# Const-me/Whisper

Measured on AMD Instinct MI355X. Metric: audio-seconds/sec (real-time factor), ggml-medium & large, 30s chunks @1/2/4/8 GPU, higher is better.
Workload: dtype f16

## Files before the change

### whisper_amd/binding.py

```python
from __future__ import annotations

import ctypes as C
import os
from typing import Optional, Sequence

import numpy as np

from . import ggml_format as gf

_HERE = os.path.dirname(os.path.abspath(__file__))
LIB_PATH = os.path.join(_HERE, "lib", "libwhisper_hip.so")

WH_FLAG_PARITY_PV = 1
WH_FLAG_NO_GRAPH = 2
WH_FLAG_DEBUG_CAPTURE = 4
WH_FLAG_PARITY_EXACT = 8
TUNE_GEMM_8WAVE = 16
TUNE_GEMM_4WAVE = 4
TUNE_GEMM_FAST_EPI = 1
TUNE_GEMV_ROWS4, TUNE_GEMM_BIG, TUNE_GEMV_SMALLREG, TUNE_GEMM_GL, TUNE_LN_SEPARATE_BIGM, TUNE_ATTN_XCD = 2, 8, 32, 64, 128, 256
TUNE_ATTN_DEC_G, TUNE_FUSE_CROSS_Q, TUNE_GEMM_GROUP_M, TUNE_FUSE_SELF_BLOCK, TUNE_GEMV_LN_BLOCK, TUNE_GEMV_K8 = 512, 1024, 2048, 4096, 8192, 16384
TUNE_SPLIT_STREAMS, TUNE_ATTN_ENC_F, TUNE_GEMM_WIDE_EPI, TUNE_GEMM_FRAGPF, TUNE_ATTN_ENC_2SWEEP = 32768, 65536, 131072, 262144, 524288
TUNE_GEMV_ALLROWS, TUNE_GEMV_ROWGROUPS, TUNE_SELF_MFMA, TUNE_MEL_MFMA = 1048576, 2097152, 4194304, 8388608
TUNE_DECODE_SMALL, TUNE_DECODE_PREFETCH, TUNE_ATTN_DEC_NT, TUNE_ENC_SERIAL = 16777216, 33554432, 67108864, 134217728
# ... 82 lines not shown
        if os.environ.get("WH_TUNING"):
            L.wh_debug_set_tuning(int(os.environ["WH_TUNING"], 0))
        L.wh_device_info.argtypes = [i32, C.c_char_p, C.c_size_t, C.POINTER(C.c_uint64), C.POINTER(C.c_int)]
        L.wh_model_arena_bytes.restype = i64
        L.wh_model_arena_bytes.argtypes = [C.POINTER(HParamsC)]
        L.wh_model_create.argtypes = [C.POINTER(HParamsC), vp, i32, C.POINTER(vp)]
        L.wh_model_destroy.argtypes = [vp]
        L.wh_model_destroy.restype = None
        L.wh_model_set_tensor.argtypes = [vp, C.c_char_p, i32, C.POINTER(C.c_int32), i32, vp]
        L.wh_model_set_filters.argtypes = [vp, i32, i32, vp]
        L.wh_model_finalize.argtypes = [vp]
        L.wh_model_arena.argtypes = [vp, C.POINTER(vp), C.POINTER(i64)]
        L.wh_model_hparams.argtypes = [vp, C.POINTER(HParamsC)]
        L.wh_context_create.argtypes = [vp, i32, vp, C.POINTER(vp)]
        L.wh_context_create_hyp.argtypes = [vp, i32, i32, vp, C.POINTER(vp)]
        L.wh_context_bind.argtypes = [vp]
        L.wh_context_destroy.argtypes = [vp]
        L.wh_context_destroy.restype = None
        L.wh_context_set_flags.argtypes = [vp, C.c_uint32, i32]
        L.wh_context_set_audio_ctx.argtypes = [vp, i32]
        L.wh_context_memory.argtypes = [vp, C.POINTER(i64)]
        L.wh_context_synchronize.argtypes = [vp]
        L.wh_buffer_upload_async.argtypes = [vp, vp, vp, i64]
        L.wh_mel_spectrogram.argtypes = [vp, vp, i64, vp, C.POINTER(i64)]
        L.wh_encode.argtypes = [vp, vp, i32, i64, i64, vp]
        L.wh_encode_windows.argtypes = [vp, vp, i32]
        L.wh_decode.argtypes = [vp, vp, i32, i32, i32, vp, vp]
        L.wh_sample_best.argtypes = [vp, i32, i32, i32, C.POINTER(TokenDataC)]
        L.wh_beam_candidates.argtypes = [vp, i32, i32, i32, i32, C.POINTER(TokenDataC)]
        L.wh_reorder_self_cache.argtypes = [vp, i32, vp, i32]
        L.wh_debug_read.argtypes = [vp, C.c_char_p, i32, i32, vp, i64]
        L.wh_decode_greedy.argtypes = [vp, i32, vp, i32, i32, i32, i32, C.POINTER(TokenDataC)]
        L.wh_decode_window_start.argtypes = [vp, i32, vp, i32, i32, i32, i32]
        L.wh_decode_window_finish.argtypes = [vp, C.POINTER(TokenDataC)]
        L.wh_decode_window_start_ragged.argtypes = [vp, i32, vp, vp, i32, i32, i32, i32]
        L.wh_decode_window_ready.argtypes = [vp, i32, i32]
        L.wh_decode_window_continue.argtypes = [vp, i32]
        L.wh_decode_window_fetch.argtypes = [vp, i32, i32, C.POINTER(TokenDataC)]
        L.wh_mel_spectrogram_window.argtypes = [vp, vp, i64, i64, i64, i64, i32, vp]
        L.wh_mel_spectrogram_batch.argtypes = [vp, vp, i64, i64, i32, vp, i64]
        L.wh_debug_probe.argtypes = [vp, i32, i32, i32, i32, i32, i32, C.POINTER(C.c_float)]
        L.wh_profile_enable.argtypes = [vp, i32]
        L.wh_profile_read.argtypes = [vp, C.POINTER(ProfileEntryC), i32, C.POINTER(i32)]
        L.wh_op_mul_mat.argtypes = [vp, vp, vp, vp, vp, vp, i32, i32, i32]
        L.wh_op_mul_mat_gelu.argtypes = [vp, vp, vp, vp, vp, i32, i32, i32]
        L.wh_op_layer_norm.argtypes = [vp, vp, vp, vp, vp, i32, i32]
        L.wh_op_flash_attention.argtypes = [vp, vp, vp, vp, vp, i32, i32, i32]
        L.wh_op_soft_max.argtypes = [vp, vp, i32, i32]
        L.wh_op_decoder_attention.argtypes = [vp, vp, vp, vp, vp, i32, i32, i32, i32, i32, i32, i32, i32, i32]
        L.wh_op_decoder_cross_attention.argtypes = [vp, vp, vp, vp, vp, vp, C.c_float, vp, vp, vp, i32, i32, i32, i32, i32]
        L.wh_op_vocab_soft_max.argtypes = [vp, vp, vp, i32, i32]
        L.wh_op_sample_best.argtypes = [vp, vp, i32, i32, i32, i32, i32, i32, i32, i32, vp]
        L.wh_op_beam_candidates.argtypes = [vp, vp, i32, i32, i32, i32, i32, i32, i32, i32, i32, vp]
        L.wh_op_reorder_self_cache.argtypes = [vp, vp, vp, vp, vp, vp, vp, i32, i32, i32, i32, i32, i32]
        L.wh_lang_detect.argtypes = [vp, i32, vp, vp]
        L.wh_model_lang_count.argtypes = [vp]
        L.wh_op_lang_probs.argtypes = [vp, vp, i32, i32, i32, i32, vp, vp]
        L.wh_resample_out_len.argtypes = [i32, i64, C.POINTER(i64)]
        L.wh_resample.argtypes = [vp, vp, i32, i32, i32, i32, i64, vp, i64, i64]
        L.wh_resample_host.argtypes = [vp, i32, i32, i32, i32, i64, vp, i64, i64]
        L.wh_resample_host_multi.argtypes = [vp, i32, i32, vp, i32, i32, i64, vp, vp, i64]
        L.wh_resample_taps.argtypes = [i32, C.POINTER(C.c_int32), C.POINTER(C.c_int32), C.POINTER(C.c_int32), C.POINTER(C.c_int32), vp, i64]
        L.wh_vad_frame_count.argtypes = [i64, C.POINTER(i64)]
        L.wh_vad_features.argtypes = [vp, vp, i64, vp]
        L.wh_vad_features_host.argtypes = [vp, i64, vp]
        L.wh_dequantize.argtypes = [vp, i32, vp, i64, vp]
        L.wh_model_set_alignment_heads.argtypes = [vp, vp, i32]
        L.wh_align_tokens.argtypes = [vp, i32, vp, vp, vp, i32, vp]
        L.wh_op_align_matrix.argtypes = [vp, vp, i64, i32, vp, i64, i32, i32, i32, vp, i32, vp, vp, i32, i32, i32, vp, vp]
        L.wh_op_dtw.argtypes = [vp, vp, i32, i32, i32, vp, vp, vp]
        _lib = L
    return _lib


def check(rc: int):
    if rc != 0:
        raise WhisperHipError("libwhisper_hip rc=%d: %s" % (rc, lib().wh_last_error().decode(errors="replace")))


def set_option(name: str, value: int):
    check(lib().wh_debug_set_option(name.encode(), int(value)))


OPTION_DEFAULTS = {"dec_tile": 0, "dec_depth": 0, "dec_wide_rows": 1, "dec_deep_rows": 0, "vocab_decrows": 0, "enc_chunk": 128, "self_fuse_max_rows": 32, "self_nq": 0, "self_wave_min_rows": 32, "enc_exp": 5, "exact_enc_layers": -1, "exact_alt_order": 0, "gemm_mf16": 1, "dec_lds": 1, "dec_lds_ks": 2, "dec_split": 1, "cross_mfma": 1, "vocab_lds": 1, "beam_regs": 1, "reorder_group": 1, "gemm_big_min_rows": 8192, "resample_lds_phases": 853}


def get_option(name: str) -> int:
    v = C.c_int(0)
    check(lib().wh_debug_get_option(name.encode(), C.byref(v)))
    return v.value


def get_option_default(name: str) -> int:
    return OPTION_DEFAULTS[name]


def device_count() -> int:
    return lib().wh_device_count()


def device_info(device: int = 0):
    name = C.create_string_buffer(256)
    mem = C.c_uint64()
    cus = C.c_int()
    check(lib().wh_device_info(device, name, 256, C.byref(mem), C.byref(cus)))
    return dict(name=name.value.decode(), total_mem=mem.value, compute_units=cus.value)


def _hp_c(hp: gf.HParams) -> HParamsC:
    return HParamsC(*hp.as_list())


def arena_bytes(hp: gf.HParams) -> int:
    n = lib().wh_model_arena_bytes(C.byref(_hp_c(hp)))
    if n < 0:
        check(-1)
    return int(n)


class HipModel:

    def __init__(self, hp: gf.HParams, arena_ptr: int = 0, already_filled: bool = False, keepalive=None):
        self.hp = hp
        self.handle = C.c_void_p()
        self._keepalive = keepalive
        check(lib().wh_model_create(C.byref(_hp_c(hp)), C.c_void_p(arena_ptr) if arena_ptr else None, int(already_filled),
                                    C.byref(self.handle)))

    @classmethod
    def from_ggml(cls, model: gf.GgmlModel, arena_ptr: int = 0, keepalive=None) -> "HipModel":
        m = cls(model.hparams, arena_ptr, False, keepalive)
        L = lib()
        filt = np.ascontiguousarray(model.filters, np.float32)
        check(L.wh_model_set_filters(m.handle, filt.shape[0], filt.shape[1], filt.ctypes.data_as(C.c_void_p)))
        for name, a in model.tensors.items():
            if isinstance(a, gf.QTensor):
                blocks = np.ascontiguousarray(a.blocks, np.uint8)
                ne = (C.c_int32 * len(a.shape))(*reversed(a.shape))
                check(L.wh_model_set_tensor(m.handle, name.encode(), len(a.shape), ne, gf.GGML_TYPES[a.qtype], blocks.ctypes.data_as(C.c_void_p)))
                continue
            a = np.ascontiguousarray(a)
            ne = (C.c_int32 * a.ndim)(*reversed(a.shape))
            check(L.wh_model_set_tensor(m.handle, name.encode(), a.ndim, ne, int(a.dtype == np.float16), a.ctypes.data_as(C.c_void_p)))
        check(L.wh_model_finalize(m.handle))
        return m

    @classmethod
    def from_file(cls, path: str) -> "HipModel":
        return cls.from_ggml(gf.read_model(path))

    def lang_count(self) -> int:
        n = lib().wh_model_lang_count(self.handle)
        if n < 0:
            check(n)
        return n

    def set_alignment_heads(self, pairs):
        a = np.ascontiguousarray(pairs, np.int32).reshape(-1, 2)
        check(lib().wh_model_set_alignment_heads(self.handle, a.ctypes.data_as(C.c_void_p) if len(a) else None, len(a)))

    def arena(self):
        p = C.c_void_p()
        n = C.c_int64()
        check(lib().wh_model_arena(self.handle, C.byref(p), C.byref(n)))
        return p.value, n.value

    def close(self):
# ... 327 lines not shown
```

### whisper_amd/csrc/attn_enc.hip

```cpp
#include "kernels.h"
#include <type_traits>

namespace wh
{
	namespace
	{
		constexpr int AQ = 64;
		constexpr int AWAVES = 8;
		constexpr int QSTRIDE = 72;
		constexpr int OSTRIDE = 65;
		constexpr int ATT_LDS_BYTES = AQ * QSTRIDE * 2 + 2 * AWAVES * AQ * 4 + AWAVES * AQ * 8 + 4 * AQ * OSTRIDE * 4;

		template<int KT>
		__global__ void __launch_bounds__( 512, 2 ) attentionEnc( const f16* __restrict__ q, const f16* __restrict__ k,
			const f16* __restrict__ vT, f16* __restrict__ out, int heads, int T, int Tpad, int nQ, int xcdRemap )
		{
			extern __shared__ __attribute__( ( aligned( 16 ) ) ) unsigned char smem[];
			f16* const ldsQ = (f16*)smem;
			float* const redMax = (float*)( smem + AQ * QSTRIDE * 2 );
			float* const redInv = redMax + AWAVES * AQ;
			double* const redSum = (double*)( redInv + AWAVES * AQ );
			float* const obuf = (float*)( redSum + AWAVES * AQ );

			const int tid = threadIdx.x;
// ... 594 lines not shown
			issueV( 0, 0 );
			for( int t = 0; t < nTiles; t++ )
			{
				const int buf = t & 1;
				asm volatile( "s_waitcnt vmcnt(0)" ::: "memory" );
				__syncthreads();
				if( t + 1 < nTiles )
				{
					issueK( t + 1, buf ^ 1 );
					issueV( t + 1, buf ^ 1 );
				}
				const f16* const kt = ldsK + buf * F_TILE;
				const f16* const vt = ldsV + buf * F_TILE;
	#pragma unroll
				for( int st = 0; st < 4; st++ )
				{
					const f32x16 S = scores( kt, st, t );
					f16x8 P[ 2 ];
	#pragma unroll
					for( int r = 0; r < 16; r += 2 )
					{
						typedef _Float16 h2 __attribute__( ( ext_vector_type( 2 ) ) );
						typedef unsigned short u16x2 __attribute__( ( ext_vector_type( 2 ) ) );
						const h2 hd = { (f16)( S[ r ] - mx ), (f16)( S[ r + 1 ] - mx ) };
						if constexpr( MODE == 0 )
						{
							u16x2 mag = __builtin_bit_cast( u16x2, __builtin_bit_cast( unsigned, hd ) & 0x7FFF7FFFu );
							const u16x2 lim = { (unsigned short)EXP_TABLE_LIMIT, (unsigned short)EXP_TABLE_LIMIT };
							mag = __builtin_elementwise_min( mag, lim );
							P[ r >> 3 ][ r & 7 ] = ldsTab[ mag[ 0 ] ];
							P[ r >> 3 ][ ( r & 7 ) + 1 ] = ldsTab[ mag[ 1 ] ];
						}
						else
						{
							typedef float f2 __attribute__( ( ext_vector_type( 2 ) ) );
							constexpr float L2E = 1.44269504088896340736f;
							const h2 hp = __builtin_convertvector( f2{ S[ r ] - mx, S[ r + 1 ] - mx }, h2 );
							const f2 e = { __builtin_amdgcn_exp2f( __builtin_fmaf( (float)hp[ 0 ], L2E, 0.0f ) ), __builtin_amdgcn_exp2f( __builtin_fmaf( (float)hp[ 1 ], L2E, 0.0f ) ) };
							const h2 eh = __builtin_convertvector( e, h2 );
							P[ r >> 3 ][ r & 7 ] = eh[ 0 ];
							P[ r >> 3 ][ ( r & 7 ) + 1 ] = eh[ 1 ];
						}
					}
					sum += (double)sumP( P );
	#pragma unroll
					for( int half = 0; half < 2; half++ )
					{
						const int kb = st * 2 + half;
	#pragma unroll
						for( int ddt = 0; ddt < 2; ddt++ )
						{
							const f16x8 vf = *(const f16x8*)( vt + ( ( kb * 2 + ddt ) * 64 + lane ) * 8 );
							O[ ddt ] = __builtin_amdgcn_mfma_f32_32x32x16_f16( vf, P[ half ], O[ ddt ], 0, 0, 0 );
						}
					}
				}
			}
			sum += __shfl_xor( sum, 32, 64 );
			const float invSum = (float)( 1.0 / sum );
	#pragma unroll
			for( int a = 0; a < 2; a++ )
	#pragma unroll
				for( int r = 0; r < 16; r++ ) O[ a ][ r ] *= invSum;
			if( qRow < T )
			{
				const int b = bh / heads, h = bh - b * heads;
				f16* const o = out + ( (long long)b * T + qRow ) * ( heads * HEAD_DIM ) + h * HEAD_DIM;
	#pragma unroll
				for( int ddt = 0; ddt < 2; ddt++ )
	#pragma unroll
					for( int g4 = 0; g4 < 4; g4++ )
					{
						f16x4 pk;
	#pragma unroll
						for( int e = 0; e < 4; e++ ) pk[ e ] = (f16)O[ ddt ][ 4 * g4 + e ];
						*(f16x4*)( o + ddt * 32 + 8 * g4 + 4 * hi ) = pk;
					}
			}
		}

		constexpr int W_NBUF = 4;
		constexpr int W_LDS_BYTES = 2 * W_NBUF * F_TILE * 2;
		constexpr float W_LAZY = 4.0f;
		template<int NG, bool ONLINE, bool NOARG = false>
		__global__ void __launch_bounds__( 1024 / NG, NG == 1 ? 4 : 2 ) attentionEncW( const f16* __restrict__ q, const f16* __restrict__ k,
			const f16* __restrict__ vT, f16* __restrict__ out, int heads, int T, int Tpad, int nQ, int xcdRemap )
		{
			extern __shared__ __attribute__( ( aligned( 16 ) ) ) unsigned char smemW[];
			f16* const ldsK = (f16*)smemW;
			f16* const ldsV = ldsK + W_NBUF * F_TILE;
			typedef __attribute__( ( address_space( 3 ) ) ) void* LdsPtr;
			typedef const __attribute__( ( address_space( 1 ) ) ) void* GlobalPtr;
			typedef _Float16 h2 __attribute__( ( ext_vector_type( 2 ) ) );
			typedef float f2 __attribute__( ( ext_vector_type( 2 ) ) );
			constexpr float L2E = 1.44269504088896340736f;

			const int tid = threadIdx.x;
			const int lane = tid & 63;
			const int wave = tid >> 6;
			const int hi = lane >> 5;
			const int c = lane & 31;
			int bh, qb;
			{
				const int L = blockIdx.x;
				if( xcdRemap )
				{
					const int kIdx = L >> 3;
					bh = ( L & 7 ) + 8 * ( kIdx / nQ );
					qb = kIdx % nQ;
				}
				else
				{
					bh = L / nQ;
					qb = L - bh * nQ;
				}
			}
			const f16* const Q = q + (long long)bh * T * HEAD_DIM;
			const f16* const K = k + (long long)bh * T * HEAD_DIM;
			const f16* const VT = vT + (long long)bh * HEAD_DIM * Tpad;
			const int nTiles = ( T + FK - 1 ) / FK;
			int qRow[ NG ];
			f16x8 qf[ NG ][ 4 ];
	#pragma unroll
			for( int g = 0; g < NG; g++ )
			{
				qRow[ g ] = qb * TQ + ( wave * NG + g ) * 32 + c;
				const int qr = qRow[ g ] < T ? qRow[ g ] : T - 1;
	#pragma unroll
				for( int kk = 0; kk < 4; kk++ )
				{
					qf[ g ][ kk ] = *(const f16x8*)( Q + (long long)qr * HEAD_DIM + kk * 16 + hi * 8 );
	#pragma unroll
					for( int j = 0; j < 8; j++ ) qf[ g ][ kk ][ j ] = qf[ g ][ kk ][ j ] * (f16)0.125f;
				}
			}
			auto issueK = [ & ]( int t, int buf )
			{
	#pragma unroll
				for( int i = 0; i < NG; i++ )
				{
					const int row = ( wave * NG + i ) * 8 + ( lane >> 3 );
					const int cl = ( lane & 7 ) ^ ( ( row >> 1 ) & 7 );
					int key = t * FK + row;
					key = key < T ? key : T - 1;
					__builtin_amdgcn_global_load_lds( (GlobalPtr)( K + (long long)key * HEAD_DIM + cl * 8 ),
						(LdsPtr)( ldsK + buf * F_TILE + ( wave * NG + i ) * 512 ), 16, 0, 0 );
				}
			};
			auto issueV = [ & ]( int t, int buf )
			{
	#pragma unroll
				for( int i = 0; i < NG; i++ )
					__builtin_amdgcn_global_load_lds( (GlobalPtr)( VT + (long long)t * F_TILE + ( wave * NG + i ) * 512 + lane * 8 ),
						(LdsPtr)( ldsV + buf * F_TILE + ( wave * NG + i ) * 512 ), 16, 0, 0 );
			};
			auto waitTile = [ & ]( int t, auto per )
			{
				constexpr int P = decltype( per )::value;
				const int younger = min( W_NBUF - 2, nTiles - 1 - t );
				if( younger >= 2 )
				{
					if constexpr( P == 2 ) asm volatile( "s_waitcnt vmcnt(4)" ::: "memory" );
					else asm volatile( "s_waitcnt vmcnt(8)" ::: "memory" );
				}
				else if( younger == 1 )
				{
					if constexpr( P == 2 ) asm volatile( "s_waitcnt vmcnt(2)" ::: "memory" );
// ... 29 lines not shown
			auto sumP = [ & ]( const f16x8 ( &P )[ 2 ] ) -> float
			{
				const h2 ones = { (f16)1.0f, (f16)1.0f };
				float part = 0.0f;
	#pragma unroll
				for( int h = 0; h < 2; h++ )
	#pragma unroll
					for( int j = 0; j < 8; j += 2 )
						part = __builtin_amdgcn_fdot2( h2{ P[ h ][ j ], P[ h ][ j + 1 ] }, ones, part, false );
				return part;
			};
			auto expTile = [ & ]( const f32x16& S, float mref, f16x8 ( &P )[ 2 ] )
			{
	#pragma unroll
				for( int r = 0; r < 16; r += 2 )
				{
					f2 e;
					if constexpr( NOARG )
					{
						const float mL = mref * L2E;
						e = f2{ __builtin_amdgcn_exp2f( __builtin_fmaf( S[ r ], L2E, -mL ) ), __builtin_amdgcn_exp2f( __builtin_fmaf( S[ r + 1 ], L2E, -mL ) ) };
					}
					else
					{
						const h2 hd = __builtin_convertvector( f2{ S[ r ] - mref, S[ r + 1 ] - mref }, h2 );
						e = f2{ __builtin_amdgcn_exp2f( __builtin_fmaf( (float)hd[ 0 ], L2E, 0.0f ) ), __builtin_amdgcn_exp2f( __builtin_fmaf( (float)hd[ 1 ], L2E, 0.0f ) ) };
					}
					const h2 eh = __builtin_convertvector( e, h2 );
					P[ r >> 3 ][ r & 7 ] = eh[ 0 ];
					P[ r >> 3 ][ ( r & 7 ) + 1 ] = eh[ 1 ];
				}
			};

			float mx[ NG ];
	#pragma unroll
			for( int g = 0; g < NG; g++ ) mx[ g ] = -INFINITY;
			if constexpr( !ONLINE )
			{
	#pragma unroll
				for( int i = 0; i < W_NBUF - 1; i++ )
					if( i < nTiles ) issueK( i, i );
				for( int t = 0; t < nTiles; t++ )
				{
					waitTile( t, std::integral_constant<int, NG>{} );
					__syncthreads();
					if( t + W_NBUF - 1 < nTiles ) issueK( t + W_NBUF - 1, ( t + W_NBUF - 1 ) % W_NBUF );
					const f16* const kt = ldsK + ( t % W_NBUF ) * F_TILE;
					auto body = [ & ]( auto last )
					{
	#pragma unroll
						for( int st = 0; st < 4; st++ )
						{
							f32x16 S[ NG ];
							scores( kt, st, t, last, S );
	#pragma unroll
							for( int g = 0; g < NG; g++ )
	#pragma unroll
								for( int r = 0; r < 16; r++ ) mx[ g ] = fmaxf( mx[ g ], S[ g ][ r ] );
						}
					};
					if( t == nTiles - 1 ) body( std::true_type{} ); else body( std::false_type{} );
				}
	#pragma unroll
				for( int g = 0; g < NG; g++ ) mx[ g ] = fmaxf( mx[ g ], __shfl_xor( mx[ g ], 32, 64 ) );
				__syncthreads();
			}

			double sum[ NG ];
			float sumF[ NG ];
			f32x16 O[ NG ][ 2 ];
	#pragma unroll
			for( int g = 0; g < NG; g++ )
			{
				sum[ g ] = 0.0;
				sumF[ g ] = 0.0f;
	#pragma unroll
				for( int a = 0; a < 2; a++ )
	#pragma unroll
					for( int r = 0; r < 16; r++ ) O[ g ][ a ][ r ] = 0.0f;
			}
	#pragma unroll
			for( int i = 0; i < W_NBUF - 1; i++ )
				if( i < nTiles ) { issueK( i, i ); issueV( i, i ); }
			for( int t = 0; t < nTiles; t++ )
			{
				waitTile( t, std::integral_constant<int, 2 * NG>{} );
				__syncthreads();
				if( t + W_NBUF - 1 < nTiles )
				{
					issueK( t + W_NBUF - 1, ( t + W_NBUF - 1 ) % W_NBUF );
					issueV( t + W_NBUF - 1, ( t + W_NBUF - 1 ) % W_NBUF );
				}
				const f16* const kt = ldsK + ( t % W_NBUF ) * F_TILE;
				const f16* const vt = ldsV + ( t % W_NBUF ) * F_TILE;
				auto body = [ & ]( auto last )
				{
	#pragma unroll
					for( int st = 0; st < 4; st++ )
					{
						f32x16 S[ NG ];
						scores( kt, st, t, last, S );
						if constexpr( ONLINE )
						{
							float tm[ NG ];
							bool raise = false;
	#pragma unroll
							for( int g = 0; g < NG; g++ )
							{
								tm[ g ] = S[ g ][ 0 ];
	#pragma unroll
								for( int r = 1; r < 16; r++ ) tm[ g ] = fmaxf( tm[ g ], S[ g ][ r ] );
								tm[ g ] = fmaxf( tm[ g ], __shfl_xor( tm[ g ], 32, 64 ) );
								raise = raise || tm[ g ] > mx[ g ] + W_LAZY;
							}
							if( __any( raise ) )
							{
	#pragma unroll
								for( int g = 0; g < NG; g++ )
								{
									const float mNew = tm[ g ] > mx[ g ] + W_LAZY ? tm[ g ] : mx[ g ];
									const float f = __builtin_amdgcn_exp2f( ( mx[ g ] - mNew ) * L2E );
									mx[ g ] = mNew;
									sumF[ g ] *= f;
	#pragma unroll
									for( int a = 0; a < 2; a++ )
	#pragma unroll
										for( int r = 0; r < 16; r++ ) O[ g ][ a ][ r ] *= f;
								}
							}
						}
						f16x8 P[ NG ][ 2 ];
	#pragma unroll
						for( int g = 0; g < NG; g++ )
						{
							expTile( S[ g ], mx[ g ], P[ g ] );
							if constexpr( ONLINE ) sumF[ g ] += sumP( P[ g ] );
							else sum[ g ] += (double)sumP( P[ g ] );
						}
	#pragma unroll
						for( int half = 0; half < 2; half++ )
						{
							const int kb = st * 2 + half;
	#pragma unroll
							for( int ddt = 0; ddt < 2; ddt++ )
							{
								const f16x8 vf = *(const f16x8*)( vt + ( ( kb * 2 + ddt ) * 64 + lane ) * 8 );
	#pragma unroll
								for( int g = 0; g < NG; g++ ) O[ g ][ ddt ] = __builtin_amdgcn_mfma_f32_32x32x16_f16( vf, P[ g ][ half ], O[ g ][ ddt ], 0, 0, 0 );
							}
						}
					}
				};
				if( t == nTiles - 1 ) body( std::true_type{} ); else body( std::false_type{} );
			}
	#pragma unroll
			for( int g = 0; g < NG; g++ )
			{
				if constexpr( ONLINE ) sum[ g ] = (double)sumF[ g ];
				sum[ g ] += __shfl_xor( sum[ g ], 32, 64 );
				const float invSum = (float)( 1.0 / sum[ g ] );
				if( qRow[ g ] < T )
				{
					const int b = bh / heads, h = bh - b * heads;
					f16* const o = out + ( (long long)b * T + qRow[ g ] ) * ( heads * HEAD_DIM ) + h * HEAD_DIM;
	#pragma unroll
					for( int ddt = 0; ddt < 2; ddt++ )
	#pragma unroll
						for( int g4 = 0; g4 < 4; g4++ )
						{
							f16x4 pk;
	#pragma unroll
							for( int e = 0; e < 4; e++ ) pk[ e ] = (f16)( O[ g ][ ddt ][ 4 * g4 + e ] * invSum );
							*(f16x4*)( o + ddt * 32 + 8 * g4 + 4 * hi ) = pk;
						}
				}
			}
		}

		template<int NG, bool ONLINE, bool NOARG = false>
		int launchEncWideT( const f16* q, const f16* k, const f16* vT, f16* out, int batch, int heads, int T, int Tpad, hipStream_t stream )
		{
			static PerDeviceOnce once;
			if( const int onceDev = once.needed(); onceDev >= 0 )
			{
				WH_HIP( hipFuncSetAttribute( (const void*)attentionEncW<NG, ONLINE, NOARG>, hipFuncAttributeMaxDynamicSharedMemorySize, W_LDS_BYTES ) );
				once.mark( onceDev );
			}
			const int nQ = ( T + TQ - 1 ) / TQ, BH = batch * heads;
			const int xcdRemap = ( BH % 8 ) == 0 && ( g_tuning & TUNE_ATTN_XCD ) ? 1 : 0;
			hipLaunchKernelGGL( ( attentionEncW<NG, ONLINE, NOARG> ), dim3( nQ * BH ), dim3( 1024 / NG ), W_LDS_BYTES, stream, q, k, vT, out, heads, T, Tpad, nQ, xcdRemap );
			WH_HIP( hipGetLastError() );
			return 0;
		}
		int launchEncWide( const f16* q, const f16* k, const f16* vT, f16* out, int batch, int heads, int T, int Tpad, int mode, hipStream_t stream )
		{
			if( mode == 5 ) return launchEncWideT<2, true, true>( q, k, vT, out, batch, heads, T, Tpad, stream );
			if( mode == 3 ) return launchEncWideT<2, true>( q, k, vT, out, batch, heads, T, Tpad, stream );
			return launchEncWideT<2, false>( q, k, vT, out, batch, heads, T, Tpad, stream );
		}

		int launchEncTable( const f16* q, const f16* k, const f16* vT, f16* out, int batch, int heads, int T, int Tpad, const f16* expTab, hipStream_t stream )
		{
			static PerDeviceOnce once;
			if( const int onceDev = once.needed(); onceDev >= 0 )
			{
				WH_HIP( hipFuncSetAttribute( (const void*)attentionEncT<0>, hipFuncAttributeMaxDynamicSharedMemorySize, T_LDS_BYTES ) );
				WH_HIP( hipFuncSetAttribute( (const void*)attentionEncT<1>, hipFuncAttributeMaxDynamicSharedMemorySize, T_LDS_BYTES - T_TABLE_HALFS * 2 ) );
				once.mark( onceDev );
			}
			const int nQ = ( T + TQ - 1 ) / TQ, BH = batch * heads;
			const int xcdRemap = ( BH % 8 ) == 0 && ( g_tuning & TUNE_ATTN_XCD ) ? 1 : 0;
			if( g_opt.encExp == 2 || g_opt.encExp == 3 || g_opt.encExp == 5 ) return launchEncWide( q, k, vT, out, batch, heads, T, Tpad, g_opt.encExp, stream );
			if( g_opt.encExp == 1 )
				hipLaunchKernelGGL( attentionEncT<1>, dim3( nQ * BH ), dim3( 1024 ), T_LDS_BYTES - T_TABLE_HALFS * 2, stream, q, k, vT, out, expTab, heads, T, Tpad, nQ, xcdRemap );
			else
			hipLaunchKernelGGL( attentionEncT<0>, dim3( nQ * BH ), dim3( 1024 ), T_LDS_BYTES, stream, q, k, vT, out, expTab, heads, T, Tpad, nQ, xcdRemap );
			WH_HIP( hipGetLastError() );
			return 0;
		}

		int launchEncF( const f16* q, const f16* k, const f16* vT, f16* out, int batch, int heads, int T, int Tpad, bool exactP, hipStream_t stream )
		{
			static PerDeviceOnce once;
			if( const int onceDev = once.needed(); onceDev >= 0 )
			{
				WH_HIP( hipFuncSetAttribute( (const void*)attentionEncF<false>, hipFuncAttributeMaxDynamicSharedMemorySize, F_LDS_BYTES ) );
				WH_HIP( hipFuncSetAttribute( (const void*)attentionEncF<true>, hipFuncAttributeMaxDynamicSharedMemorySize, F_LDS_BYTES ) );
				once.mark( onceDev );
			}
			const int nQ = ( T + FQ - 1 ) / FQ, BH = batch * heads;
			const int xcdRemap = ( BH % 8 ) == 0 && ( g_tuning & TUNE_ATTN_XCD ) ? 1 : 0;
			const bool two = !exactP && ( g_tuning & TUNE_ATTN_ENC_2SWEEP );
			if( two )
				hipLaunchKernelGGL( attentionEncF<true>, dim3( nQ * BH ), dim3( 512 ), F_LDS_BYTES, stream, q, k, vT, out, heads, T, Tpad, nQ, xcdRemap );
			else
				hipLaunchKernelGGL( attentionEncF<false>, dim3( nQ * BH ), dim3( 512 ), F_LDS_BYTES, stream, q, k, vT, out, heads, T, Tpad, nQ, xcdRemap );
			WH_HIP( hipGetLastError() );
			return 0;
		}

		template<int KT>
		int launchEncT( const f16* q, const f16* k, const f16* vT, f16* out, int batch, int heads, int T, int Tpad, hipStream_t stream )
		{
			static PerDeviceOnce once;
			if( const int onceDev = once.needed(); onceDev >= 0 )
			{
				WH_HIP( hipFuncSetAttribute( (const void*)attentionEnc<KT>, hipFuncAttributeMaxDynamicSharedMemorySize, ATT_LDS_BYTES ) );
				once.mark( onceDev );
			}
			const int nQ = ( T + AQ - 1 ) / AQ, BH = batch * heads;
			const int xcdRemap = ( BH % 8 ) == 0 && ( g_tuning & TUNE_ATTN_XCD ) ? 1 : 0;
			hipLaunchKernelGGL( attentionEnc<KT>, dim3( nQ * BH ), dim3( 512 ), ATT_LDS_BYTES, stream, q, k, vT, out, heads, T, Tpad, nQ, xcdRemap );
			WH_HIP( hipGetLastError() );
			return 0;
		}
	}

	int attentionInit() { return 0; }

	int launchAttentionEnc( const f16* q, const f16* k, const f16* vT, f16* out, int batch, int heads, int T, int Tpad, bool exactP, const f16* expTab,
		hipStream_t stream )
	{
		if( T <= 0 || T > 1536 || Tpad < ( ( T + 255 ) / 256 ) * 256 || ( Tpad & 7 ) != 0 )
		{
			setError( "attentionEnc: need 0 < T <= 1536 and Tpad >= roundup(T, 256)" );
			return -1;
		}
		if( expTab && !exactP && ( g_tuning & TUNE_ATTN_ENC_TABLE ) && ( g_tuning & TUNE_ATTN_ENC_F ) && ( g_tuning & TUNE_ATTN_ENC_2SWEEP ) &&
			( ( ( T + TQ - 1 ) / TQ ) * batch * heads >= 256 || ( g_tuning & TUNE_ATTN_ENC_TABLE_ANY ) ) )
			return launchEncTable( q, k, vT, out, batch, heads, T, Tpad, expTab, stream );
		if( g_tuning & TUNE_ATTN_ENC_F ) return launchEncF( q, k, vT, out, batch, heads, T, Tpad, exactP, stream );
		switch( ( T + 255 ) / 256 )
		{
		case 1: return launchEncT<1>( q, k, vT, out, batch, heads, T, Tpad, stream );
		case 2: return launchEncT<2>( q, k, vT, out, batch, heads, T, Tpad, stream );
		case 3: return launchEncT<3>( q, k, vT, out, batch, heads, T, Tpad, stream );
		case 4: return launchEncT<4>( q, k, vT, out, batch, heads, T, Tpad, stream );
		case 5: return launchEncT<5>( q, k, vT, out, batch, heads, T, Tpad, stream );
// ... 5 lines not shown
```

### whisper_amd/csrc/kernels.h

```cpp
#pragma once
#include "common.h"

namespace wh
{
	enum eTuning : unsigned
	{
		TUNE_GEMV_ROWS4 = 2,
		TUNE_GEMM_4WAVE = 4,
		TUNE_GEMM_FAST_EPI = 1,
		TUNE_GEMM_8WAVE = 16,
		TUNE_GEMM_BIG = 8,
		TUNE_GEMV_SMALLREG = 32,
		TUNE_GEMM_GL = 64,
		TUNE_LN_SEPARATE_BIGM = 128,
		TUNE_ATTN_XCD = 256,
		TUNE_ATTN_DEC_G = 512,
		TUNE_FUSE_CROSS_Q = 1024,
		TUNE_FUSE_SELF_BLOCK = 4096,
		TUNE_GEMV_LN_BLOCK = 8192,
		TUNE_GEMV_K8 = 16384,
		TUNE_SPLIT_STREAMS = 32768,
		TUNE_ATTN_ENC_F = 65536,
		TUNE_GEMM_WIDE_EPI = 131072,
		TUNE_GEMM_FRAGPF = 262144,
		TUNE_ATTN_ENC_2SWEEP = 524288,
		TUNE_MEL_MFMA = 8388608,
		TUNE_SELF_MFMA = 4194304,
		TUNE_GEMV_ALLROWS = 1048576,
		TUNE_GEMV_ROWGROUPS = 2097152,
		TUNE_GEMM_GROUP_M = 2048,
		TUNE_ATTN_DEC_NT = 67108864,
		TUNE_DECODE_SMALL = 16777216,
		TUNE_DECODE_PREFETCH = 33554432,
		TUNE_ATTN_ENC_TABLE = 268435456,
		TUNE_ATTN_ENC_TABLE_ANY = 1073741824,
		TUNE_SAMPLE_SPREAD = 2147483648u,
		TUNE_GEMV_MT8 = 536870912,
		TUNE_ENC_SERIAL = 134217728,
		TUNE_DEFAULT = TUNE_GEMM_FAST_EPI | TUNE_GEMM_8WAVE | TUNE_GEMV_ROWS4 | TUNE_GEMV_SMALLREG | TUNE_GEMM_BIG | TUNE_GEMM_GL | TUNE_LN_SEPARATE_BIGM | TUNE_ATTN_XCD | TUNE_ATTN_DEC_G | TUNE_FUSE_CROSS_Q | TUNE_GEMM_GROUP_M | TUNE_FUSE_SELF_BLOCK | TUNE_GEMV_K8 | TUNE_ATTN_ENC_F | TUNE_GEMM_WIDE_EPI | TUNE_GEMM_FRAGPF | TUNE_ATTN_ENC_2SWEEP | TUNE_GEMV_ALLROWS | TUNE_GEMV_ROWGROUPS | TUNE_SELF_MFMA | TUNE_MEL_MFMA | TUNE_DECODE_SMALL | TUNE_ATTN_DEC_NT | TUNE_ATTN_ENC_TABLE
	};
	extern unsigned g_tuning;

	struct Options
	{
		int decTile = 0;
		int decDepth = 0;
		int decWideRows = 1;
		int decDeepRows = 0;
		int vocabDecRows = 0;
		int encChunk = 128;
		int selfFuseMaxRows = 32;
		int selfNq = 0;
		int exactEncLayers = -1;
		int encExp = 5;
		int encAblate = 0;
		int exactAltOrder = 0;
		int decLds = 1;
		int decLdsKs = 2;
		int decSplit = 1;
		int crossMfma = 1;
		int vocabLds = 1;
		int beamRegs = 1;
		int reorderGroup = 1;
		int gemmBigMinRows = 8192;
		int gemmMf16 = 1;
		int resampleLdsPhases = 853;
		int selfWaveMinRows = 32;
	};
	extern Options g_opt;

	enum eEpilogue : int
	{
		EPI_F32 = 0,
		EPI_F16_GELU,
		EPI_CONV2,
		EPI_QKV_ENC,
		EPI_CROSS_KV,
		EPI_QKV_DEC,
		EPI_Q_DEC,
	};

	struct GemmArgs
	{
		const f16* A;
		const f16* W;
		int M, N, K;
		int lda, Mb;
		long long aBatchStride;
		int epi;
		const float* bias;
		const float* res;
		float* out32;
		f16* out16;
		int ldc;
		long long cBatchStride;
		const float* pe;
		float scale;
		f16* q;
		f16* k;
		f16* v;
		int T, Tpad, H, B;
		int nTok, nPast, textCtx;
		const int* nPastDev;
		const float* lnX;
		const float* lnW;
		const float* lnB;
		int wideEpi;
		int groupM;
		float* splitScratch;
		int cuLimit;
	};

	int launchGemm( const GemmArgs& a, hipStream_t stream );
	int launchGemmSkinny( const GemmArgs& a, hipStream_t stream );
	int launchGemv( const GemmArgs& a, hipStream_t stream );
	constexpr int GEMV_FUSED_MAX_ROWS = 128;
	constexpr int GEMV_MAX_ROWS = 512;
	int launchGemmVariant( const GemmArgs& a, int variant, hipStream_t stream );
	int gemmInit();

	int launchLayerNorm( const float* x, const float* w, const float* b, f16* out, int rows, int d, hipStream_t stream );
	struct MelWindow
	{
		const float* mel;
		long long len;
		int offset, reserved;
	};
	int launchMelToConvInput( const float* mel, long long melStride, long long melLen, const int* melOffsets, const MelWindow* wins,
		f16* x16, long long xBatchStride, int nMels, int T, int batch, hipStream_t stream );
	int launchEmbed( const int* tokens, const f16* te, const float* pe, float* x, int rows, int nTok, int nPast, const int* nPastDev, int d,
		int nVocab, int nTextCtx, hipStream_t stream );
	int launchSoftMaxRows( float* x, int rows, int cols, hipStream_t stream );

	int launchExactMulMat( const f16* W, int N, int K, const float* X, long long ldx, int M, float* out, long long ldo, const float* bias, float scale, bool useScale,
		const f16* geluTab, const float* residual, long long ldr, hipStream_t stream );
	int launchExactNorm( const float* x, const float* w, const float* b, float* out, int rows, int n, hipStream_t stream );
	int launchExactConv( const f16* W, int kpad, int ic, const void* X, bool in16, long long xBatchStride, int Tin, int stride, const float* bias, const f16* geluTab,
// ... 176 lines not shown
```

### whisper_amd/csrc/options.hip

```cpp
#include "runtime.h"

namespace wh
{
	unsigned g_tuning = TUNE_DEFAULT;
	Options g_opt;
	namespace
	{
		struct OptionName { const char* name; int Options::* field; };
		const OptionName g_optionNames[] = { { "dec_tile", &Options::decTile }, { "dec_depth", &Options::decDepth }, { "dec_wide_rows", &Options::decWideRows }, { "dec_deep_rows", &Options::decDeepRows }, { "vocab_decrows", &Options::vocabDecRows }, { "enc_chunk", &Options::encChunk },
			{ "self_fuse_max_rows", &Options::selfFuseMaxRows }, { "self_nq", &Options::selfNq }, { "self_wave_min_rows", &Options::selfWaveMinRows }, { "exact_enc_layers", &Options::exactEncLayers }, { "exact_alt_order", &Options::exactAltOrder }, { "enc_exp", &Options::encExp }, { "enc_ablate", &Options::encAblate }, { "gemm_mf16", &Options::gemmMf16 }, { "dec_lds", &Options::decLds }, { "dec_lds_ks", &Options::decLdsKs }, { "dec_split", &Options::decSplit }, { "vocab_lds", &Options::vocabLds }, { "beam_regs", &Options::beamRegs }, { "reorder_group", &Options::reorderGroup }, { "gemm_big_min_rows", &Options::gemmBigMinRows }, { "cross_mfma", &Options::crossMfma }, { "resample_lds_phases", &Options::resampleLdsPhases } };
		const bool g_optionsFromEnv = []()
		{
			for( const OptionName& o : g_optionNames )
			{
				std::string env = "WH_OPT_";
				for( const char* p = o.name; *p; p++ ) env.push_back( (char)toupper( (unsigned char)*p ) );
				if( const char* e = getenv( env.c_str() ) )
				{
					char* end = nullptr;
					const long v = strtol( e, &end, 10 );
					if( end != e && *end == 0 && v >= -1 && v <= ( 1 << 24 ) ) g_opt.*( o.field ) = (int)v;
					else fprintf( stderr, "[wh] %s='%s' ignored (not an integer in [-1, 2^24])\n", env.c_str(), e );
				}
			}
			return true;
		}();
	}
	static thread_local std::string g_lastError;
	void setError( const std::string& s ) { g_lastError = s; }
	int hipFail( hipError_t e, const char* what, const char* file, int line )
	{
		char buf[ 512 ];
		snprintf( buf, sizeof( buf ), "HIP error %d (%s) at %s:%d: %s", (int)e, hipGetErrorString( e ), file, line, what );
		g_lastError = buf;
		return WH_E_HIP;
	}
}

extern "C" {

const char* wh_last_error( void ) { return g_lastError.c_str(); }

int wh_debug_set_tuning( uint32_t mask )
{
	g_tuning = mask;
	return 0;
}

int wh_debug_set_option( const char* name, int value )
{
	if( !name ) { setError( "debug_set_option: null name" ); return WH_E_INVALIDARG; }
	for( const OptionName& o : g_optionNames )
		if( 0 == strcmp( o.name, name ) )
		{
			if( value < -1 || value > ( 1 << 24 ) ) { setError( std::string( "option '" ) + name + "': value out of range" ); return WH_E_INVALIDARG; }
			g_opt.*( o.field ) = value;
			return 0;
		}
	setError( "debug_set_option: unknown option" );
	return WH_E_INVALIDARG;
}

int wh_debug_get_option( const char* name, int* value )
{
	if( !name || !value ) { setError( "debug_get_option: null argument" ); return WH_E_INVALIDARG; }
	for( const OptionName& o : g_optionNames )
		if( 0 == strcmp( o.name, name ) )
		{
			*value = g_opt.*( o.field );
			return 0;
		}
	setError( "debug_get_option: unknown option" );
	return WH_E_INVALIDARG;
}

}
```

Measured before the change: 10440.

## Add software-pipelined encoder attention loop with K-fragment double buffering

Adds a SCHED=1 variant of the wide encoder attention kernel that reads the next sub-tile's K fragments from LDS while the current sub-tile's score MFMAs and softmax run, with V fragments loaded early and sched_barriers pinning the instruction order. It also exits early on the last tile once the valid sub-tiles are done, instead of computing masked ones. The aim is to hide LDS latency behind MFMA work in the encoder attention. The variant is on by default through a new enc_sched option, which costs extra registers for the double-buffered fragments and hand-written asm for the rescale step.

After: 10580 (median of 6 runs). +1.3%, better.

```diff
diff --git a/whisper_amd/binding.py b/whisper_amd/binding.py
--- a/whisper_amd/binding.py
+++ b/whisper_amd/binding.py
@@ -188,7 +188,7 @@
     check(lib().wh_debug_set_option(name.encode(), int(value)))
 
 
-OPTION_DEFAULTS = {"dec_tile": 0, "dec_depth": 0, "dec_wide_rows": 1, "dec_deep_rows": 0, "vocab_decrows": 0, "enc_chunk": 128, "self_fuse_max_rows": 32, "self_nq": 0, "self_wave_min_rows": 32, "enc_exp": 5, "exact_enc_layers": -1, "exact_alt_order": 0, "gemm_mf16": 1, "dec_lds": 1, "dec_lds_ks": 2, "dec_split": 1, "cross_mfma": 1, "vocab_lds": 1, "beam_regs": 1, "reorder_group": 1, "gemm_big_min_rows": 8192, "resample_lds_phases": 853}
+OPTION_DEFAULTS = {"dec_tile": 0, "dec_depth": 0, "dec_wide_rows": 1, "dec_deep_rows": 0, "vocab_decrows": 0, "enc_chunk": 128, "self_fuse_max_rows": 32, "self_nq": 0, "self_wave_min_rows": 32, "enc_exp": 5, "enc_sched": 1, "exact_enc_layers": -1, "exact_alt_order": 0, "gemm_mf16": 1, "dec_lds": 1, "dec_lds_ks": 2, "dec_split": 1, "cross_mfma": 1, "vocab_lds": 1, "beam_regs": 1, "reorder_group": 1, "gemm_big_min_rows": 8192, "resample_lds_phases": 853}
 
 
 def get_option(name: str) -> int:
diff --git a/whisper_amd/csrc/attn_enc.hip b/whisper_amd/csrc/attn_enc.hip
--- a/whisper_amd/csrc/attn_enc.hip
+++ b/whisper_amd/csrc/attn_enc.hip
@@ -700,7 +700,7 @@
 		constexpr int W_NBUF = 4;
 		constexpr int W_LDS_BYTES = 2 * W_NBUF * F_TILE * 2;
 		constexpr float W_LAZY = 4.0f;
-		template<int NG, bool ONLINE, bool NOARG = false>
+		template<int NG, bool ONLINE, bool NOARG = false, int SCHED = 0>
 		__global__ void __launch_bounds__( 1024 / NG, NG == 1 ? 4 : 2 ) attentionEncW( const f16* __restrict__ q, const f16* __restrict__ k,
 			const f16* __restrict__ vT, f16* __restrict__ out, int heads, int T, int Tpad, int nQ, int xcdRemap )
 		{
@@ -896,6 +896,114 @@
 	#pragma unroll
 			for( int i = 0; i < W_NBUF - 1; i++ )
 				if( i < nTiles ) { issueK( i, i ); issueV( i, i ); }
+			if constexpr( SCHED == 1 )
+			{
+				static_assert( ONLINE && NG == 2, "the scheduled loop is the one-sweep form of two query groups per wave" );
+				const int swK = ( c >> 1 ) & 7;
+				auto tile = [ & ]( int t, auto last )
+				{
+					waitTile( t, std::integral_constant<int, 2 * NG>{} );
+					__syncthreads();
+					if( t + W_NBUF - 1 < nTiles )
+					{
+						issueK( t + W_NBUF - 1, ( t + W_NBUF - 1 ) % W_NBUF );
+						issueV( t + W_NBUF - 1, ( t + W_NBUF - 1 ) % W_NBUF );
+					}
+					const f16* const kt = ldsK + ( t % W_NBUF ) * F_TILE;
+					const f16* const vt = ldsV + ( t % W_NBUF ) * F_TILE;
+					auto readK = [ & ]( int st, f16x8 ( &kf )[ 4 ] )
+					{
+		#pragma unroll
+						for( int kk = 0; kk < 4; kk++ ) kf[ kk ] = *(const f16x8*)( kt + ( st * 32 + c ) * HEAD_DIM + ( ( ( kk * 2 + hi ) ^ swK ) << 3 ) );
+					};
+					auto subTile = [ & ]( int st, auto last, const f16x8 ( &kcur )[ 4 ], f16x8 ( &knext )[ 4 ] )
+					{
+						f32x16 S[ NG ];
+		#pragma unroll
+						for( int kk = 0; kk < 4; kk++ )
+		#pragma unroll
+							for( int g = 0; g < NG; g++ ) S[ g ] = __builtin_amdgcn_mfma_f32_32x32x16_f16( kcur[ kk ], qf[ g ][ kk ], kk == 0 ? zero16 : S[ g ], 0, 0, 0 );
+						f16x8 vf[ 4 ];
+		#pragma unroll
+						for( int i = 0; i < 4; i++ ) vf[ i ] = *(const f16x8*)( vt + ( ( st * 4 + i ) * 64 + lane ) * 8 );
+						if( st + 1 < 4 ) readK( st + 1, knext );
+						__builtin_amdgcn_sched_barrier( 0 );
+						if constexpr( decltype( last )::value )
+						{
+							const int limit = T - ( t * FK + st * 32 + 4 * hi );
+		#pragma unroll
+							for( int r = 0; r < 16; r++ )
+							{
+								const bool in = ( r & 3 ) + 8 * ( r >> 2 ) < limit;
+		#pragma unroll
+								for( int g = 0; g < NG; g++ ) S[ g ][ r ] = in ? S[ g ][ r ] : -3.0e38f;
+							}
+						}
+						float tm[ NG ];
+						bool raise = false;
+		#pragma unroll
+						for( int g = 0; g < NG; g++ )
+						{
+							tm[ g ] = S[ g ][ 0 ];
+		#pragma unroll
+							for( int r = 1; r < 16; r++ ) tm[ g ] = fmaxf( tm[ g ], S[ g ][ r ] );
+							const unsigned tb = __builtin_bit_cast( unsigned, tm[ g ] );
+							const auto sw2 = __builtin_amdgcn_permlane32_swap( tb, tb, false, false );
+							tm[ g ] = fmaxf( tm[ g ], __builtin_bit_cast( float, hi ? sw2[ 0 ] : sw2[ 1 ] ) );
+							raise = raise || tm[ g ] > mx[ g ] + W_LAZY;
+						}
+						if( __any( raise ) )
+						{
+		#pragma unroll
+							for( int g = 0; g < NG; g++ )
+							{
+								const float mNew = tm[ g ] > mx[ g ] + W_LAZY ? tm[ g ] : mx[ g ];
+								float f = __builtin_amdgcn_exp2f( ( mx[ g ] - mNew ) * L2E );
+								mx[ g ] = mNew;
+								sumF[ g ] *= f;
+								__builtin_amdgcn_sched_barrier( 0 );
+								asm volatile( "s_nop 7" : "+v"( f ) );
+		#pragma unroll
+								for( int a = 0; a < 2; a++ )
+		#pragma unroll
+									for( int r = 0; r < 16; r++ )
+									{
+										float x = O[ g ][ a ][ r ];
+										asm volatile( "v_mul_f32 %0, %0, %1" : "+v"( x ) : "v"( f ) );
+										O[ g ][ a ][ r ] = x;
+									}
+							}
+							__builtin_amdgcn_sched_barrier( 0 );
+						}
+						f16x8 P[ NG ][ 2 ];
+		#pragma unroll
+						for( int g = 0; g < NG; g++ )
+						{
+							expTile( S[ g ], mx[ g ], P[ g ] );
+							sumF[ g ] += sumP( P[ g ] );
+						}
+		#pragma unroll
+						for( int half = 0; half < 2; half++ )
+		#pragma unroll
+							for( int ddt = 0; ddt < 2; ddt++ )
+		#pragma unroll
+								for( int g = 0; g < NG; g++ ) O[ g ][ ddt ] = __builtin_amdgcn_mfma_f32_32x32x16_f16( vf[ half * 2 + ddt ], P[ g ][ half ], O[ g ][ ddt ], 0, 0, 0 );
+					};
+					const int nValid = decltype( last )::value ? ( T - t * FK + 31 ) >> 5 : 4;
+					f16x8 kA[ 4 ], kB[ 4 ];
+					readK( 0, kA );
+					subTile( 0, last, kA, kB );
+					if( nValid < 2 ) return;
+					subTile( 1, last, kB, kA );
+					if( nValid < 3 ) return;
+					subTile( 2, last, kA, kB );
+					if( nValid < 4 ) return;
+					subTile( 3, last, kB, kA );
+				};
+				for( int t = 0; t < nTiles - 1; t++ ) tile( t, std::false_type{} );
+				tile( nTiles - 1, std::true_type{} );
+			}
+			else
 			for( int t = 0; t < nTiles; t++ )
 			{
 				waitTile( t, std::integral_constant<int, 2 * NG>{} );
@@ -991,23 +1099,33 @@
 			}
 		}
 
-		template<int NG, bool ONLINE, bool NOARG = false>
+		template<int NG, bool ONLINE, bool NOARG = false, int SCHED = 0>
 		int launchEncWideT( const f16* q, const f16* k, const f16* vT, f16* out, int batch, int heads, int T, int Tpad, hipStream_t stream )
 		{
 			static PerDeviceOnce once;
 			if( const int onceDev = once.needed(); onceDev >= 0 )
 			{
-				WH_HIP( hipFuncSetAttribute( (const void*)attentionEncW<NG, ONLINE, NOARG>, hipFuncAttributeMaxDynamicSharedMemorySize, W_LDS_BYTES ) );
+				WH_HIP( hipFuncSetAttribute( (const void*)attentionEncW<NG, ONLINE, NOARG, SCHED>, hipFuncAttributeMaxDynamicSharedMemorySize, W_LDS_BYTES ) );
 				once.mark( onceDev );
 			}
 			const int nQ = ( T + TQ - 1 ) / TQ, BH = batch * heads;
 			const int xcdRemap = ( BH % 8 ) == 0 && ( g_tuning & TUNE_ATTN_XCD ) ? 1 : 0;
-			hipLaunchKernelGGL( ( attentionEncW<NG, ONLINE, NOARG> ), dim3( nQ * BH ), dim3( 1024 / NG ), W_LDS_BYTES, stream, q, k, vT, out, heads, T, Tpad, nQ, xcdRemap );
+			hipLaunchKernelGGL( ( attentionEncW<NG, ONLINE, NOARG, SCHED> ), dim3( nQ * BH ), dim3( 1024 / NG ), W_LDS_BYTES, stream, q, k, vT, out, heads, T, Tpad, nQ, xcdRemap );
 			WH_HIP( hipGetLastError() );
 			return 0;
 		}
 		int launchEncWide( const f16* q, const f16* k, const f16* vT, f16* out, int batch, int heads, int T, int Tpad, int mode, hipStream_t stream )
 		{
+			if( g_opt.encSched != 0 && g_opt.encSched != 1 )
+			{
+				setError( "attentionEnc: option enc_sched must be 0 or 1" );
+				return -1;
+			}
+			if( g_opt.encSched == 1 )
+			{
+				if( mode == 5 ) return launchEncWideT<2, true, true, 1>( q, k, vT, out, batch, heads, T, Tpad, stream );
+				if( mode == 3 ) return launchEncWideT<2, true, false, 1>( q, k, vT, out, batch, heads, T, Tpad, stream );
+			}
 			if( mode == 5 ) return launchEncWideT<2, true, true>( q, k, vT, out, batch, heads, T, Tpad, stream );
 			if( mode == 3 ) return launchEncWideT<2, true>( q, k, vT, out, batch, heads, T, Tpad, stream );
 			return launchEncWideT<2, false>( q, k, vT, out, batch, heads, T, Tpad, stream );
diff --git a/whisper_amd/csrc/kernels.h b/whisper_amd/csrc/kernels.h
--- a/whisper_amd/csrc/kernels.h
+++ b/whisper_amd/csrc/kernels.h
@@ -53,6 +53,7 @@
 		int selfNq = 0;
 		int exactEncLayers = -1;
 		int encExp = 5;
+		int encSched = 1;
 		int encAblate = 0;
 		int exactAltOrder = 0;
 		int decLds = 1;
diff --git a/whisper_amd/csrc/options.hip b/whisper_amd/csrc/options.hip
--- a/whisper_amd/csrc/options.hip
+++ b/whisper_amd/csrc/options.hip
@@ -8,7 +8,7 @@
 	{
 		struct OptionName { const char* name; int Options::* field; };
 		const OptionName g_optionNames[] = { { "dec_tile", &Options::decTile }, { "dec_depth", &Options::decDepth }, { "dec_wide_rows", &Options::decWideRows }, { "dec_deep_rows", &Options::decDeepRows }, { "vocab_decrows", &Options::vocabDecRows }, { "enc_chunk", &Options::encChunk },
-			{ "self_fuse_max_rows", &Options::selfFuseMaxRows }, { "self_nq", &Options::selfNq }, { "self_wave_min_rows", &Options::selfWaveMinRows }, { "exact_enc_layers", &Options::exactEncLayers }, { "exact_alt_order", &Options::exactAltOrder }, { "enc_exp", &Options::encExp }, { "enc_ablate", &Options::encAblate }, { "gemm_mf16", &Options::gemmMf16 }, { "dec_lds", &Options::decLds }, { "dec_lds_ks", &Options::decLdsKs }, { "dec_split", &Options::decSplit }, { "vocab_lds", &Options::vocabLds }, { "beam_regs", &Options::beamRegs }, { "reorder_group", &Options::reorderGroup }, { "gemm_big_min_rows", &Options::gemmBigMinRows }, { "cross_mfma", &Options::crossMfma }, { "resample_lds_phases", &Options::resampleLdsPhases } };
+			{ "self_fuse_max_rows", &Options::selfFuseMaxRows }, { "self_nq", &Options::selfNq }, { "self_wave_min_rows", &Options::selfWaveMinRows }, { "exact_enc_layers", &Options::exactEncLayers }, { "exact_alt_order", &Options::exactAltOrder }, { "enc_exp", &Options::encExp }, { "enc_sched", &Options::encSched }, { "enc_ablate", &Options::encAblate }, { "gemm_mf16", &Options::gemmMf16 }, { "dec_lds", &Options::decLds }, { "dec_lds_ks", &Options::decLdsKs }, { "dec_split", &Options::decSplit }, { "vocab_lds", &Options::vocabLds }, { "beam_regs", &Options::beamRegs }, { "reorder_group", &Options::reorderGroup }, { "gemm_big_min_rows", &Options::gemmBigMinRows }, { "cross_mfma", &Options::crossMfma }, { "resample_lds_phases", &Options::resampleLdsPhases } };
 		const bool g_optionsFromEnv = []()
 		{
 			for( const OptionName& o : g_optionNames )
```
